# eladb3/SViT

Measured on NVIDIA B200. Metric: clips/sec (16x224^2, bf16) SViT forward, higher is better.
Workload: dtype bf16

## Files before the change

svit_b200/csrc/pool_ln_tiled.cu:

```cuda
#include <cstdlib>
#include <type_traits>

#include "tc_common.cuh"

namespace {

constexpr int PD = 96;
constexpr int TAPS = 27;

struct Geom {
  int B, h, T, H, W, Ho, Wo, O, s;
  int64_t in_bs, in_ts, in_hs;
};

__device__ __forceinline__ float lo_f(uint32_t w) { return __uint_as_float(w << 16); }
__device__ __forceinline__ float hi_f(uint32_t w) { return __uint_as_float(w & 0xffff0000u); }
__device__ __forceinline__ uint32_t pack2(float a, float b) {
  __nv_bfloat162 v = __floats2bfloat162_rn(a, b);
  return *reinterpret_cast<uint32_t*>(&v);
}
__device__ __forceinline__ float half_sum(float v) {
  const unsigned mask = 0xffffu << (threadIdx.x & 16);
#pragma unroll
  for (int o = 8; o > 0; o >>= 1) v += __shfl_xor_sync(mask, v, o);
// ... 392 lines not shown
      if (ho0 + srow >= g.Ho || nvalid < 0) nvalid = 0;
      const int64_t row0 = ((int64_t)bh * Nout + 1 + (int64_t)(ho0 + srow) * g.Wo + wo0 + scol) * PD;
      optr = reinterpret_cast<uint32_t*>(out + row0) + wd;
      if (SAVE) pptr = reinterpret_cast<uint32_t*>(pre + row0) + wd;
    }
    if (g.T == 1) {
      step(R0{}, EONLY{}, 0);
    } else {
      step(R0{}, EFIRST{}, 0);
      int tp = 1;
      for (; tp + 3 <= g.T - 1; tp += 3) {
        step(R1{}, EMID{}, tp);
        step(R2{}, EMID{}, tp + 1);
        step(R0{}, EMID{}, tp + 2);
      }
      const int rem = g.T - 1 - tp;
      if (rem == 0) {
        step(R1{}, ELAST{}, tp);
      } else if (rem == 1) {
        step(R1{}, EMID{}, tp);
        step(R2{}, ELAST{}, tp + 1);
      } else {
        step(R1{}, EMID{}, tp);
        step(R2{}, EMID{}, tp + 1);
        step(R0{}, ELAST{}, tp + 2);
      }
    }
  }

  {
    float2* stg = reinterpret_cast<float2*>(ring);
    long long* stg_tok = reinterpret_cast<long long*>(smem + C::NTOK * MK_PITCH * 8);
    float* sweff = aff + 2 * PD;
    const int nbh = g.B * g.h;
    bool have_weff = false;
    for (int item = gridDim.x - 1 - blockIdx.x; item < nbh; item += gridDim.x) {
      if (!have_weff) {
        if (threadIdx.x < 48) {
          float2 a = make_float2(0.f, 0.f);
#pragma unroll
          for (int tp = 0; tp < TAPS; ++tp) {
            const float f = __ldg(frac + tp);
            a.x = fmaf(sw2[tp * 48 + wd].x, f, a.x);
            a.y = fmaf(sw2[tp * 48 + wd].y, f, a.y);
          }
          sweff[2 * wd] = a.x;
          sweff[2 * wd + 1] = a.y;
        }
        have_weff = true;
      }
      const int head = item % g.h, b = item / g.h;
      const bf16* zin = in + (int64_t)b * g.in_bs + (int64_t)head * g.in_hs;
      bf16* obase = out + (int64_t)item * Nout * PD;
      for (int base = 0; base < 1 + g.O; base += C::NTOK) {
        __syncthreads();
        const int n = min(C::NTOK, 1 + g.O - base);
        for (int i = threadIdx.x; i < n * 48; i += MK_THREADS) {
          const int k = i / 48, ww = i - k * 48;
          const int r = base + k;
          const int64_t tok_in = r == 0 ? 0 : L + r;
          const uint32_t v = reinterpret_cast<const uint32_t*>(zin + tok_in * g.in_ts)[ww];
          const float sx = r == 0 ? 1.f : sweff[2 * ww], sy = r == 0 ? 1.f : sweff[2 * ww + 1];
          stg[k * MK_PITCH + ww] = make_float2(lo_f(v) * sx, hi_f(v) * sy);
          if (ww == 0) stg_tok[k] = r == 0 ? 0 : Lo + r;
        }
        __syncthreads();
        mk_ln_flush(stg, stg_tok, aff, n, eps, obase, threadIdx.x, SAVE ? pre + (int64_t)item * Nout * PD : nullptr);
      }
    }
  }
}

__global__ void __launch_bounds__(256, 4)
pool_ln_direct_kernel(const bf16* __restrict__ in, Geom g, const float* __restrict__ w, const float* __restrict__ frac,
                      const float* __restrict__ gamma, const float* __restrict__ beta, bf16* __restrict__ out, float eps,
                      int mode, bf16* __restrict__ pre) {
  __shared__ float sw[TAPS * PD];
  __shared__ float sweff[PD];
  for (int i = threadIdx.x; i < PD * TAPS; i += blockDim.x) sw[(i % TAPS) * PD + i / TAPS] = w[i];
  __syncthreads();
  for (int c = threadIdx.x; c < PD; c += blockDim.x) {
    float a = 0.f;
    for (int t = 0; t < TAPS; ++t) a += sw[t * PD + c] * frac[t];
    sweff[c] = a;
  }
  __syncthreads();
  const int lane = threadIdx.x & 31, l16 = lane & 15;
  float gm[6], bt[6];
  load_affine(gamma, beta, l16, gm, bt);
  const int64_t Lo = (int64_t)g.T * g.Ho * g.Wo, L = (int64_t)g.T * g.H * g.W;
  const int64_t Nout = 1 + Lo + g.O;
  const int64_t per_bh = mode == 0 ? Nout : (int64_t)1 + g.O;
  const int64_t total = (int64_t)g.B * g.h * per_bh;
  const int64_t hw_per_grid = (int64_t)gridDim.x * (blockDim.x >> 4);
  for (int64_t i = (int64_t)blockIdx.x * (blockDim.x >> 4) + (threadIdx.x >> 4); i < total; i += hw_per_grid) {
    const int64_t r = i % per_bh;
    const int64_t tok = mode == 0 ? r : (r == 0 ? 0 : Lo + r);
    const int head = (int)((i / per_bh) % g.h);
    const int b = (int)(i / (per_bh * g.h));
    const bf16* zin = in + (int64_t)b * g.in_bs + (int64_t)head * g.in_hs;
    float v[6] = {0.f, 0.f, 0.f, 0.f, 0.f, 0.f};
    if (tok == 0 || tok > Lo) {
      const uint32_t* p = reinterpret_cast<const uint32_t*>(zin + (tok == 0 ? 0 : (tok - Lo + L)) * g.in_ts);
#pragma unroll
      for (int j = 0; j < 3; ++j) {
        const uint32_t wd = p[l16 + 16 * j];
        const int c = 2 * (l16 + 16 * j);
        v[2 * j] = lo_f(wd) * (tok == 0 ? 1.f : sweff[c]);
        v[2 * j + 1] = hi_f(wd) * (tok == 0 ? 1.f : sweff[c + 1]);
      }
    } else {
      const int64_t pp = tok - 1;
      const int wo = (int)(pp % g.Wo), ho = (int)((pp / g.Wo) % g.Ho), to = (int)(pp / ((int64_t)g.Wo * g.Ho));
#pragma unroll
      for (int kt = 0; kt < 3; ++kt) {
        const int t = to - 1 + kt;
        if (t < 0 || t >= g.T) continue;
        uint32_t xw[9][3];
#pragma unroll
        for (int kh = 0; kh < 3; ++kh) {
          const int hh = ho * g.s - 1 + kh;
#pragma unroll
          for (int kw = 0; kw < 3; ++kw) {
            const int ww = wo * g.s - 1 + kw;
            const bool ok = hh >= 0 && hh < g.H && ww >= 0 && ww < g.W;
            const uint32_t* q = reinterpret_cast<const uint32_t*>(
                zin + (ok ? (1 + ((int64_t)t * g.H + hh) * g.W + ww) * g.in_ts : 0));
#pragma unroll
            for (int j = 0; j < 3; ++j) xw[kh * 3 + kw][j] = ok ? __ldg(q + l16 + 16 * j) : 0u;
          }
        }
#pragma unroll
        for (int tap = 0; tap < 9; ++tap) {
          const float* wr = sw + (kt * 9 + tap) * PD;
#pragma unroll
          for (int j = 0; j < 3; ++j) {
            const float2 f = *reinterpret_cast<const float2*>(wr + 2 * (l16 + 16 * j));
            v[2 * j] = fmaf(lo_f(xw[tap][j]), f.x, v[2 * j]);
            v[2 * j + 1] = fmaf(hi_f(xw[tap][j]), f.y, v[2 * j + 1]);
          }
        }
      }
    }
    uint32_t* dst = reinterpret_cast<uint32_t*>(out + (((int64_t)b * g.h + head) * Nout + tok) * PD);
    if (pre) {
      uint32_t* pd = reinterpret_cast<uint32_t*>(pre + (((int64_t)b * g.h + head) * Nout + tok) * PD);
#pragma unroll
      for (int j = 0; j < 3; ++j) pd[l16 + 16 * j] = pack2(v[2 * j], v[2 * j + 1]);
    }
    ln_store(v, gm, bt, eps, dst, l16);
  }
}

}

#ifdef SVIT_TIMELINE
extern "C" int svit_debug_pool_timeline(void* device_buffer) {
  unsigned long long* p = (unsigned long long*)device_buffer;
  return (int)cudaMemcpyToSymbol(g_pool_dbg, &p, sizeof(p));
}
#endif

namespace {
template <int SV, int SPRV, bool PERSIST, bool SAVE>
int launch_march(const void* in, int64_t in_bs, int64_t in_ts, const Geom& g, const float* conv_w, const float* tap_frac,
                 const float* gamma, const float* beta, void* out, float eps, cudaStream_t st, void* pre) {
  using C = MkCfg<SV, SPRV>;
  svit_tmap_encode_fn enc = svit_get_tmap_encode();
  if (!enc) return SVIT_ENOTSUP;
  CUtensorMap tm;
  cuuint64_t dims[5] = {(cuuint64_t)g.h * PD, (cuuint64_t)g.W, (cuuint64_t)g.H, (cuuint64_t)g.T, (cuuint64_t)g.B};
  cuuint64_t strides[4] = {(cuuint64_t)in_ts * 2, (cuuint64_t)g.W * in_ts * 2, (cuuint64_t)g.H * g.W * in_ts * 2, (cuuint64_t)in_bs * 2};
  cuuint32_t box[5] = {PD, (cuuint32_t)C::IW, (cuuint32_t)C::IH, 1, 1};
  cuuint32_t estr[5] = {1, 1, 1, 1, 1};
  const bf16* base = (const bf16*)in + in_ts;
  if (enc(&tm, CU_TENSOR_MAP_DATA_TYPE_BFLOAT16, 5, const_cast<bf16*>(base), dims, strides, box, estr,
          CU_TENSOR_MAP_INTERLEAVE_NONE, CU_TENSOR_MAP_SWIZZLE_NONE, CU_TENSOR_MAP_L2_PROMOTION_L2_256B,
          CU_TENSOR_MAP_FLOAT_OOB_FILL_NONE) != CUDA_SUCCESS)
    return SVIT_EINVAL;
  auto kern = pool_ln_march_kernel<SV, SPRV, PERSIST, SAVE>;
  static SvitDevOnce configured;
  if (configured.need()) {
    SVIT_CUDA(cudaFuncSetAttribute(kern, cudaFuncAttributeMaxDynamicSharedMemorySize, C::SMEM));
    configured.done();
  }
  const int tiles = ((g.Wo + C::TW - 1) / C::TW) * ((g.Ho + C::ROWS - 1) / C::ROWS);
  const int64_t ncols = (int64_t)tiles * g.h * g.B;
  if (ncols > (1ll << 30)) return SVIT_EINVAL;
  int64_t grid = PERSIST ? (int64_t)svit_num_sms() * 2 : ncols;
  if (grid > ncols) grid = ncols;
  kern<<<(unsigned)grid, MK_THREADS, C::SMEM, st>>>(tm, (const bf16*)in, g, conv_w, tap_frac, gamma, beta, (bf16*)out, eps,
                                                    tiles, (int)ncols, (bf16*)pre);
  SVIT_CHECK_LAUNCH();
  return 0;
}
}

int svit_pool_ln_fwd_bf16(const void* in, int64_t in_bs, int64_t in_ts, int64_t in_hs, const float* conv_w,
                          const float* tap_frac, const float* gamma, const float* beta, void* out, int B, int h, int T,
                          int H, int W, int O, int s, float eps, cudaStream_t st, void* pre) {
  Geom g;
  g.B = B; g.h = h; g.T = T; g.H = H; g.W = W; g.O = O; g.s = s;
  g.Ho = (H - 1) / s + 1; g.Wo = (W - 1) / s + 1;
  g.in_bs = in_bs; g.in_ts = in_ts; g.in_hs = in_hs;
  const int sms = svit_num_sms();
  const bool tma_ok = (s == 1 || s == 2) && (in_ts % 8 == 0) && (in_bs % 8 == 0) && in_hs == PD && (T * H * W) > 0 &&
                      ((reinterpret_cast<uintptr_t>(in) & 15) == 0) && ((reinterpret_cast<uintptr_t>(out) & 15) == 0);
  if (tma_ok) {
    static const int mode = []() { const char* e = getenv("SVIT_POOL_PERSIST"); return e ? atoi(e) : -1; }();
    const bool wide = s == 1 && g.Wo > 7;
    const int64_t cols_s2 = (int64_t)((g.Wo + 6) / 7) * ((g.Ho + 3) / 4) * h * B;
    const bool persist = mode < 0 ? (s == 2 && cols_s2 >= (int64_t)sms * 12) : mode != 0;
#define MARCH(SV, SPRV)                                                                                               \
  (pre ? (persist ? launch_march<SV, SPRV, true, true>(in, in_bs, in_ts, g, conv_w, tap_frac, gamma, beta, out, eps, st, pre)    \
                  : launch_march<SV, SPRV, false, true>(in, in_bs, in_ts, g, conv_w, tap_frac, gamma, beta, out, eps, st, pre)) \
       : (persist ? launch_march<SV, SPRV, true, false>(in, in_bs, in_ts, g, conv_w, tap_frac, gamma, beta, out, eps, st, nullptr) \
                  : launch_march<SV, SPRV, false, false>(in, in_bs, in_ts, g, conv_w, tap_frac, gamma, beta, out, eps, st, nullptr)))
    if (s == 2) return MARCH(2, 2);
    if (!wide) return MARCH(1, 1);
    return MARCH(1, 2);
#undef MARCH
  }
  const int64_t total = (int64_t)B * h * (1 + (int64_t)T * g.Ho * g.Wo + O);
  int64_t blocks = (total + 15) / 16;
  if (blocks > (int64_t)sms * 16) blocks = (int64_t)sms * 16;
  if (blocks < 1) blocks = 1;
  pool_ln_direct_kernel<<<(unsigned)blocks, 256, 0, st>>>((const bf16*)in, g, conv_w, tap_frac, gamma, beta, (bf16*)out, eps, 0, (bf16*)pre);
  SVIT_CHECK_LAUNCH();
  return 0;
}
```

svit_b200/csrc/stream_bf16.cu:

```cuda
#include "common.cuh"

namespace {

__device__ __forceinline__ void unpack4(uint2 v, float f[4]) {
  f[0] = __uint_as_float(v.x << 16); f[1] = __uint_as_float(v.x & 0xffff0000u);
  f[2] = __uint_as_float(v.y << 16); f[3] = __uint_as_float(v.y & 0xffff0000u);
}
__device__ __forceinline__ uint32_t pack2(float a, float b) {
  __nv_bfloat162 v = __floats2bfloat162_rn(a, b);
  return *reinterpret_cast<uint32_t*>(&v);
}

template <int G, int NQ>
__global__ void __launch_bounds__(256) layernorm_bf16_kernel(const bf16* __restrict__ x, const float* __restrict__ gamma,
                                                             const float* __restrict__ beta, bf16* __restrict__ y,
                                                             float* __restrict__ mean_out, float* __restrict__ rstd_out,
                                                             int64_t rows, float eps) {
  constexpr int C = 4 * G * NQ;
  const int lg = threadIdx.x % G;
  const int64_t group = ((int64_t)blockIdx.x * blockDim.x + threadIdx.x) / G;
  const int64_t ngroups = (int64_t)gridDim.x * blockDim.x / G;
  float gm[NQ][4], bt[NQ][4];
#pragma unroll
  for (int q = 0; q < NQ; ++q) {
    const float4 g4 = *reinterpret_cast<const float4*>(gamma + 4 * (lg + G * q));
    const float4 b4 = *reinterpret_cast<const float4*>(beta + 4 * (lg + G * q));
    gm[q][0] = g4.x; gm[q][1] = g4.y; gm[q][2] = g4.z; gm[q][3] = g4.w;
    bt[q][0] = b4.x; bt[q][1] = b4.y; bt[q][2] = b4.z; bt[q][3] = b4.w;
  }
  const int64_t iters = (rows + ngroups - 1) / ngroups;
  for (int64_t it = 0; it < iters; ++it) {
    const int64_t row = group + it * ngroups;
    const bool ok = row < rows;
    float v[NQ][4];
    float s = 0.f;
#pragma unroll
    for (int q = 0; q < NQ; ++q) {
      uint2 raw = make_uint2(0u, 0u);
      if (ok) raw = *reinterpret_cast<const uint2*>(x + row * C + 4 * (lg + G * q));
      unpack4(raw, v[q]);
      s += v[q][0] + v[q][1] + v[q][2] + v[q][3];
    }
#pragma unroll
    for (int o = G / 2; o > 0; o >>= 1) s += __shfl_xor_sync(0xffffffffu, s, o);
    const float mean = s * (1.f / C);
    float qq = 0.f;
#pragma unroll
    for (int q = 0; q < NQ; ++q)
#pragma unroll
      for (int i = 0; i < 4; ++i) {
        v[q][i] -= mean;
        qq += v[q][i] * v[q][i];
      }
#pragma unroll
    for (int o = G / 2; o > 0; o >>= 1) qq += __shfl_xor_sync(0xffffffffu, qq, o);
    const float rstd = rsqrtf(qq * (1.f / C) + eps);
    if (ok) {
#pragma unroll
      for (int q = 0; q < NQ; ++q) {
        uint2 o2;
        o2.x = pack2(v[q][0] * rstd * gm[q][0] + bt[q][0], v[q][1] * rstd * gm[q][1] + bt[q][1]);
        o2.y = pack2(v[q][2] * rstd * gm[q][2] + bt[q][2], v[q][3] * rstd * gm[q][3] + bt[q][3]);
        *reinterpret_cast<uint2*>(y + row * C + 4 * (lg + G * q)) = o2;
      }
      if (lg == 0 && mean_out) {
        mean_out[row] = mean;
        rstd_out[row] = rstd;
      }
    }
  }
}

template <typename TI>
__global__ void __launch_bounds__(256) im2col_rows_kernel(const TI* __restrict__ x, bf16* __restrict__ cols, int Cin, int T,
                                                          int H, int W, int To, int Ho, int Wo, int kt, int kh, int kw,
                                                          int st, int sh, int sw, int pt, int ph, int pw, int Kpad, int RW) {
  extern __shared__ __align__(16) unsigned char smem_raw[];
  const int R = Cin * kt * kh;
  bf16* rows = reinterpret_cast<bf16*>(smem_raw);
  int* koff = reinterpret_cast<int*>(smem_raw + (((size_t)R * RW * 2 + 15) & ~size_t(15)));
  const int ho = blockIdx.x % Ho, to = (blockIdx.x / Ho) % To, b = blockIdx.x / (Ho * To);
  const int K = R * kw;
  for (int k = threadIdx.x; k < Kpad; k += blockDim.x) koff[k] = k < K ? (k / kw) * RW + (k % kw) : -1;
  for (int i = threadIdx.x; i < R * RW; i += blockDim.x) {
    const int r = i / RW, col = i % RW;
    const int dh = r % kh, dt = (r / kh) % kt, c = r / (kh * kt);
    const int t = to * st - pt + dt, hh = ho * sh - ph + dh, ww = col - pw;
    float v = 0.f;
    if (t >= 0 && t < T && hh >= 0 && hh < H && ww >= 0 && ww < W)
      v = to_f(x[((((int64_t)b * Cin + c) * T + t) * H + hh) * W + ww]);
    rows[i] = __float2bfloat16_rn(v);
  }
  __syncthreads();
  const int cpr = Kpad >> 3;
  bf16* obase = cols + ((((int64_t)b * To + to) * Ho + ho) * Wo) * Kpad;
  const unsigned short* rs = reinterpret_cast<const unsigned short*>(rows);
  for (int i = threadIdx.x; i < Wo * cpr; i += blockDim.x) {
    const int wo = i / cpr, q = i % cpr;
    const int base = wo * sw;
    unsigned short e[8];
#pragma unroll
    for (int u = 0; u < 8; ++u) {
      const int off = koff[q * 8 + u];
      e[u] = off < 0 ? (unsigned short)0 : rs[off + base];
    }
    uint4 o;
    o.x = e[0] | ((uint32_t)e[1] << 16); o.y = e[2] | ((uint32_t)e[3] << 16);
    o.z = e[4] | ((uint32_t)e[5] << 16); o.w = e[6] | ((uint32_t)e[7] << 16);
    *reinterpret_cast<uint4*>(obase + (int64_t)wo * Kpad + q * 8) = o;
  }
}

constexpr int IM_HALO = 4;
__global__ void __launch_bounds__(256) im2col_rows_vec_kernel(const bf16* __restrict__ x, bf16* __restrict__ cols, int Cin,
                                                              int T, int H, int W, int To, int Ho, int Wo, int kt, int kh,
                                                              int kw, int st, int sh, int sw, int pt, int ph, int pw,
                                                              int Kpad, int RW) {
  extern __shared__ __align__(16) unsigned char smem_raw[];
  unsigned short* rows = reinterpret_cast<unsigned short*>(smem_raw);
  const int R = Cin * kt * kh, K = R * kw;
  const int ho = blockIdx.x % Ho, to = (blockIdx.x / Ho) % To, b = blockIdx.x / (Ho * To);
  const int cpr = Kpad >> 3, wchunks = W >> 3;
  for (int i = threadIdx.x; i < R * (wchunks + 2); i += blockDim.x) {
    const int r = i / (wchunks + 2), j = i % (wchunks + 2) - 1;
    unsigned short* dst = rows + r * RW;
    if (j < 0) {
      *reinterpret_cast<uint2*>(dst) = make_uint2(0u, 0u);
    } else if (j == wchunks) {
      *reinterpret_cast<uint2*>(dst + IM_HALO + W) = make_uint2(0u, 0u);
    } else {
      const int dh = r % kh, dt = (r / kh) % kt, c = r / (kh * kt);
      const int t = to * st - pt + dt, hh = ho * sh - ph + dh;
      uint4 v = make_uint4(0u, 0u, 0u, 0u);
      if (t >= 0 && t < T && hh >= 0 && hh < H)
        v = __ldg(reinterpret_cast<const uint4*>(x + ((((int64_t)b * Cin + c) * T + t) * H + hh) * W + 8 * j));
      uint2* d2 = reinterpret_cast<uint2*>(dst + IM_HALO + 8 * j);
      d2[0] = make_uint2(v.x, v.y);
      d2[1] = make_uint2(v.z, v.w);
    }
  }
  const int q = threadIdx.x % cpr, w_first = threadIdx.x / cpr, w_step = blockDim.x / cpr;
  int off[8];
#pragma unroll
  for (int u = 0; u < 8; ++u) {
    const int k = q * 8 + u;
    off[u] = k < K ? (k / kw) * RW + (k % kw) + IM_HALO - pw : -1;
  }
  __syncthreads();
  bf16* obase = cols + ((((int64_t)b * To + to) * Ho + ho) * Wo) * Kpad + q * 8;
  for (int wo = w_first; wo < Wo; wo += w_step) {
    const int base = wo * sw;
    unsigned short e[8];
#pragma unroll
    for (int u = 0; u < 8; ++u) e[u] = off[u] < 0 ? (unsigned short)0 : rows[off[u] + base];
    uint4 o;
    o.x = e[0] | ((uint32_t)e[1] << 16); o.y = e[2] | ((uint32_t)e[3] << 16);
    o.z = e[4] | ((uint32_t)e[5] << 16); o.w = e[6] | ((uint32_t)e[7] << 16);
    *reinterpret_cast<uint4*>(obase + (int64_t)wo * Kpad) = o;
  }
}

template <bool IDX>
__global__ void __launch_bounds__(256) skip_maxpool_bf16_kernel(const bf16* __restrict__ x, bf16* __restrict__ y,
                                                                uint8_t* __restrict__ idx, int B, int C,
                                                                int T_, int H, int W, int Ho, int Wo, int O, int s) {
  const int C8 = C >> 3;
  const int64_t Lin = (int64_t)T_ * H * W, Lout = (int64_t)T_ * Ho * Wo;
  const int64_t Nin = 1 + Lin + O, Nout = 1 + Lout + O;
  const int64_t total = (int64_t)B * Nout * C8;
  for (int64_t i = (int64_t)blockIdx.x * blockDim.x + threadIdx.x; i < total; i += (int64_t)gridDim.x * blockDim.x) {
    const int c8 = (int)(i % C8);
    const int64_t r = i / C8;
    const int64_t tok = r % Nout;
    const int b = (int)(r / Nout);
    const bf16* xb = x + (int64_t)b * Nin * C + c8 * 8;
    uint4 o;
    if (tok == 0) {
      o = *reinterpret_cast<const uint4*>(xb);
    } else if (tok > Lout) {
      o = *reinterpret_cast<const uint4*>(xb + (tok - Lout + Lin) * C);
    } else {
      const int64_t p = tok - 1;
      const int wo = (int)(p % Wo), ho = (int)((p / Wo) % Ho), t = (int)(p / ((int64_t)Wo * Ho));
      uint4 taps[9];
      bool ok[9];
#pragma unroll
      for (int dh = 0; dh < 3; ++dh)
#pragma unroll
        for (int dw = 0; dw < 3; ++dw) {
          const int hh = ho * s - 1 + dh, ww = wo * s - 1 + dw;
          ok[dh * 3 + dw] = hh >= 0 && hh < H && ww >= 0 && ww < W;
          taps[dh * 3 + dw] = ok[dh * 3 + dw]
              ? *reinterpret_cast<const uint4*>(xb + (1 + ((int64_t)t * H + hh) * W + ww) * C) : make_uint4(0, 0, 0, 0);
        }
      float m[8];
      uint32_t win[8];
#pragma unroll
      for (int u = 0; u < 8; ++u) { m[u] = -INFINITY; win[u] = 0u; }
#pragma unroll
      for (int k = 0; k < 9; ++k)
        if (ok[k]) {
          const uint32_t wv[4] = {taps[k].x, taps[k].y, taps[k].z, taps[k].w};
#pragma unroll
          for (int u = 0; u < 4; ++u) {
            const float a = __uint_as_float(wv[u] << 16), c = __uint_as_float(wv[u] & 0xffff0000u);
            if (a > m[2 * u] || a != a) { m[2 * u] = a; if (IDX) win[2 * u] = (uint32_t)k; }
            if (c > m[2 * u + 1] || c != c) { m[2 * u + 1] = c; if (IDX) win[2 * u + 1] = (uint32_t)k; }
          }
        }
      o.x = pack2(m[0], m[1]); o.y = pack2(m[2], m[3]); o.z = pack2(m[4], m[5]); o.w = pack2(m[6], m[7]);
      if (IDX) {
        uint2 iv;
        iv.x = win[0] | (win[1] << 8) | (win[2] << 16) | (win[3] << 24);
        iv.y = win[4] | (win[5] << 8) | (win[6] << 16) | (win[7] << 24);
        *reinterpret_cast<uint2*>(idx + ((int64_t)b * Nout + tok) * C + c8 * 8) = iv;
      }
    }
    *reinterpret_cast<uint4*>(y + ((int64_t)b * Nout + tok) * C + c8 * 8) = o;
  }
}

__global__ void __launch_bounds__(256) skip_maxpool_bwd_idx_kernel(const uint8_t* __restrict__ idx, const bf16* __restrict__ dy,
                                                                   bf16* __restrict__ dx, int B, int C, int T_, int H, int W,
                                                                   int Ho, int Wo, int O, int s) {
  const int C8 = C >> 3;
  const int64_t Lin = (int64_t)T_ * H * W, Lout = (int64_t)T_ * Ho * Wo;
  const int64_t Nin = 1 + Lin + O, Nout = 1 + Lout + O;
  const int64_t total = (int64_t)B * Nin * C8;
  for (int64_t i = (int64_t)blockIdx.x * blockDim.x + threadIdx.x; i < total; i += (int64_t)gridDim.x * blockDim.x) {
    const int c = (int)(i % C8) * 8;
    const int64_t r = i / C8;
    const int64_t tok = r % Nin;
    const int b = (int)(r / Nin);
    const bf16* dyb = dy + (int64_t)b * Nout * C + c;
    const uint8_t* ib = idx + (int64_t)b * Nout * C + c;
    bf16* o = dx + r * C + c;
    if (tok == 0) {
      *reinterpret_cast<uint4*>(o) = __ldg(reinterpret_cast<const uint4*>(dyb));
      continue;
    }
    if (tok > Lin) {
      *reinterpret_cast<uint4*>(o) = __ldg(reinterpret_cast<const uint4*>(dyb + (tok - Lin + Lout) * C));
      continue;
    }
    const int64_t p = tok - 1;
    const int w = (int)(p % W), h = (int)((p / W) % H), t = (int)(p / ((int64_t)W * H));
    float g[8] = {0.f, 0.f, 0.f, 0.f, 0.f, 0.f, 0.f, 0.f};
    for (int ho = (h - 1 + s - 1) / s; ho * s <= h + 1 && ho < Ho; ++ho) {
      if (ho < 0) continue;
      const int dh = h - (ho * s - 1);
      for (int wo = (w - 1 + s - 1) / s; wo * s <= w + 1 && wo < Wo; ++wo) {
        if (wo < 0) continue;
        const uint32_t me = (uint32_t)(dh * 3 + (w - (wo * s - 1)));
        const int64_t orow = 1 + ((int64_t)t * Ho + ho) * Wo + wo;
        const uint2 iv = __ldg(reinterpret_cast<const uint2*>(ib + orow * C));
        const uint32_t hit_lo = iv.x ^ (me * 0x01010101u), hit_hi = iv.y ^ (me * 0x01010101u);
        if (((hit_lo - 0x01010101u) & ~hit_lo & 0x80808080u) | ((hit_hi - 0x01010101u) & ~hit_hi & 0x80808080u)) {
          const uint4 dv = __ldg(reinterpret_cast<const uint4*>(dyb + orow * C));
          const uint32_t wv[4] = {dv.x, dv.y, dv.z, dv.w};
#pragma unroll
          for (int u = 0; u < 4; ++u) {
            const uint32_t b0 = ((u < 2 ? hit_lo : hit_hi) >> (16 * (u & 1))) & 0xffu;
            const uint32_t b1 = ((u < 2 ? hit_lo : hit_hi) >> (16 * (u & 1) + 8)) & 0xffu;
            if (b0 == 0u) g[2 * u] += __uint_as_float(wv[u] << 16);
            if (b1 == 0u) g[2 * u + 1] += __uint_as_float(wv[u] & 0xffff0000u);
          }
        }
      }
    }
    uint4 ov;
    ov.x = pack2(g[0], g[1]); ov.y = pack2(g[2], g[3]); ov.z = pack2(g[4], g[5]); ov.w = pack2(g[6], g[7]);
    *reinterpret_cast<uint4*>(o) = ov;
  }
}

}

extern "C" int svit_skip_maxpool_fwd_idx(const void* x, void* y, void* idx, int B, int C, int T, int H, int W, int O,
                                         int stride_hw, int dtype, void* stream) {
  if (!x || !y || !idx || stride_hw < 2 || B < 0 || O < 1) return SVIT_EINVAL;
  if (dtype != SVIT_BF16 || C % 8 ||
      ((reinterpret_cast<uintptr_t>(x) | reinterpret_cast<uintptr_t>(y)) & 15) || (reinterpret_cast<uintptr_t>(idx) & 7))
    return SVIT_ENOTSUP;
  const int Ho = (H - 1) / stride_hw + 1, Wo = (W - 1) / stride_hw + 1;
  const int64_t total = (int64_t)B * (1 + (int64_t)T * Ho * Wo + O) * (C / 8);
  if (total == 0) return 0;
  int64_t blocks = (total + 255) / 256;
  if (blocks > (int64_t)svit_num_sms() * 32) blocks = (int64_t)svit_num_sms() * 32;
  skip_maxpool_bf16_kernel<true><<<(unsigned)blocks, 256, 0, (cudaStream_t)stream>>>((const bf16*)x, (bf16*)y, (uint8_t*)idx, B, C,
                                                                                   T, H, W, Ho, Wo, O, stride_hw);
  SVIT_CHECK_LAUNCH();
  return 0;
}

extern "C" int svit_skip_maxpool_bwd_idx(const void* idx, const void* dy, void* dx, int B, int C, int T, int H, int W, int O,
                                         int stride_hw, int dtype, void* stream) {
  if (!idx || !dy || !dx || stride_hw < 2 || B < 0 || O < 1) return SVIT_EINVAL;
  if (dtype != SVIT_BF16 || C % 8 ||
      ((reinterpret_cast<uintptr_t>(dy) | reinterpret_cast<uintptr_t>(dx)) & 15) || (reinterpret_cast<uintptr_t>(idx) & 7))
    return SVIT_ENOTSUP;
  const int Ho = (H - 1) / stride_hw + 1, Wo = (W - 1) / stride_hw + 1;
  const int64_t total = (int64_t)B * (1 + (int64_t)T * H * W + O) * (C / 8);
  if (total == 0) return 0;
  int64_t blocks = (total + 255) / 256;
  if (blocks > (int64_t)svit_num_sms() * 32) blocks = (int64_t)svit_num_sms() * 32;
  skip_maxpool_bwd_idx_kernel<<<(unsigned)blocks, 256, 0, (cudaStream_t)stream>>>((const uint8_t*)idx, (const bf16*)dy, (bf16*)dx, B,
                                                                                C, T, H, W, Ho, Wo, O, stride_hw);
  SVIT_CHECK_LAUNCH();
  return 0;
}

int svit_skip_maxpool_fwd_bf16(const void* x, void* y, int B, int C, int T, int H, int W, int Ho, int Wo, int O, int s,
                               cudaStream_t st) {
  if (C % 8 || (reinterpret_cast<uintptr_t>(x) & 15) || (reinterpret_cast<uintptr_t>(y) & 15)) return 0;
  const int64_t total = (int64_t)B * (1 + (int64_t)T * Ho * Wo + O) * (C / 8);
  int64_t blocks = (total + 255) / 256;
  if (blocks > (int64_t)svit_num_sms() * 32) blocks = (int64_t)svit_num_sms() * 32;
  skip_maxpool_bf16_kernel<false><<<(unsigned)blocks, 256, 0, st>>>((const bf16*)x, (bf16*)y, nullptr, B, C, T, H, W, Ho, Wo, O, s);
  cudaError_t e = cudaGetLastError();
  return e == cudaSuccess ? 1 : 1000 + (int)e;
}

int svit_layernorm_fwd_bf16(const void* x, const float* gamma, const float* beta, void* y, float* mean, float* rstd,
                            int64_t rows, int C, float eps, cudaStream_t st) {
  if ((reinterpret_cast<uintptr_t>(x) & 7) || (reinterpret_cast<uintptr_t>(y) & 7) ||
      (reinterpret_cast<uintptr_t>(gamma) & 15) || (reinterpret_cast<uintptr_t>(beta) & 15))
    return 0;
  const int sms = svit_num_sms();
#define LN_LAUNCH(G, NQ)                                                                                           \
  {                                                                                                                \
    int64_t blocks = (rows * G + 255) / 256;                                                                       \
    if (blocks > (int64_t)sms * 16) blocks = (int64_t)sms * 16;                                                    \
    layernorm_bf16_kernel<G, NQ><<<(unsigned)blocks, 256, 0, st>>>((const bf16*)x, gamma, beta, (bf16*)y, mean, rstd, \
                                                                  rows, eps);                                      \
  }
  if (C == 96) LN_LAUNCH(8, 3)
  else if (C == 192) LN_LAUNCH(16, 3)
  else if (C == 384) LN_LAUNCH(32, 3)
  else if (C == 768) LN_LAUNCH(32, 6)
  else return 0;
#undef LN_LAUNCH
  cudaError_t e = cudaGetLastError();
  return e == cudaSuccess ? 1 : 1000 + (int)e;
}

int svit_im2col_rows(const void* x, void* cols, int B, int Cin, int T, int H, int W, int To, int Ho, int Wo, int kt, int kh,
                     int kw, int st_, int sh, int sw, int pt, int ph, int pw, int Kpad, int in_dtype, cudaStream_t st) {
  if (Kpad % 8 || (reinterpret_cast<uintptr_t>(cols) & 15)) return 0;
  const int R = Cin * kt * kh;
  const int RW = (W + 2 * pw + 1) & ~1;
  if ((Wo - 1) * sw + kw > RW) return 0;
  const size_t smem = (((size_t)R * RW * 2 + 15) & ~size_t(15)) + (size_t)Kpad * 4;
  if (smem > 200 * 1024) return 0;
  const unsigned grid = (unsigned)((int64_t)B * To * Ho);
  cudaError_t e;
  const int cpr = Kpad / 8;
  if (in_dtype == SVIT_BF16 && W % 8 == 0 && pw <= IM_HALO && cpr <= 64 && (reinterpret_cast<uintptr_t>(x) & 15) == 0) {
    const int RWv = (W + 2 * IM_HALO + 7) & ~7;
    const int threads = (256 / cpr) * cpr;
    const size_t smv = (size_t)R * RWv * 2;
    if ((Wo - 1) * sw + kw - 1 - pw < W + 4 && smv <= 200 * 1024) {
      static size_t confv = 0;
      if (smv > confv) {
        if ((e = cudaFuncSetAttribute(im2col_rows_vec_kernel, cudaFuncAttributeMaxDynamicSharedMemorySize, (int)smv)) != cudaSuccess)
          return 1000 + (int)e;
        confv = smv;
      }
      im2col_rows_vec_kernel<<<grid, threads, smv, st>>>((const bf16*)x, (bf16*)cols, Cin, T, H, W, To, Ho, Wo, kt, kh, kw, st_,
                                                         sh, sw, pt, ph, pw, Kpad, RWv);
      e = cudaGetLastError();
      return e == cudaSuccess ? 1 : 1000 + (int)e;
    }
  }
  if (in_dtype == SVIT_BF16) {
    static size_t conf = 0;
    if (smem > conf) {
      if ((e = cudaFuncSetAttribute(im2col_rows_kernel<bf16>, cudaFuncAttributeMaxDynamicSharedMemorySize, (int)smem)) != cudaSuccess)
        return 1000 + (int)e;
      conf = smem;
    }
    im2col_rows_kernel<bf16><<<grid, 256, smem, st>>>((const bf16*)x, (bf16*)cols, Cin, T, H, W, To, Ho, Wo, kt, kh, kw, st_,
                                                      sh, sw, pt, ph, pw, Kpad, RW);
  } else {
    static size_t conf = 0;
    if (smem > conf) {
      if ((e = cudaFuncSetAttribute(im2col_rows_kernel<float>, cudaFuncAttributeMaxDynamicSharedMemorySize, (int)smem)) != cudaSuccess)
        return 1000 + (int)e;
      conf = smem;
    }
    im2col_rows_kernel<float><<<grid, 256, smem, st>>>((const float*)x, (bf16*)cols, Cin, T, H, W, To, Ho, Wo, kt, kh, kw,
                                                       st_, sh, sw, pt, ph, pw, Kpad, RW);
  }
  e = cudaGetLastError();
  return e == cudaSuccess ? 1 : 1000 + (int)e;
}


template <typename OT>
__global__ void __launch_bounds__(256) normalize_u8_kernel(const uint8_t* __restrict__ in, OT* __restrict__ out, int64_t npix16,
                                                           int64_t THW, float m0, float m1, float m2, float s0, float s1,
                                                           float s2) {
  const float mean[3] = {m0, m1, m2}, sd[3] = {s0, s1, s2};
  for (int64_t i = (int64_t)blockIdx.x * blockDim.x + threadIdx.x; i < npix16; i += (int64_t)gridDim.x * blockDim.x) {
    const int64_t pix = i * 16;
    const int64_t b = pix / THW, r = pix - b * THW;
    const uint4* src = reinterpret_cast<const uint4*>(in + pix * 3);
    const uint4 q0 = __ldg(src), q1 = __ldg(src + 1), q2 = __ldg(src + 2);
    const uint32_t w[12] = {q0.x, q0.y, q0.z, q0.w, q1.x, q1.y, q1.z, q1.w, q2.x, q2.y, q2.z, q2.w};
    float v[3][16];
#pragma unroll
    for (int k = 0; k < 48; ++k) {
      const float f = (float)((w[k >> 2] >> ((k & 3) * 8)) & 255u);
      const int c = k % 3;
      v[c][k / 3] = __fdiv_rn(__fsub_rn(__fdiv_rn(f, 255.0f), mean[c]), sd[c]);
    }
#pragma unroll
    for (int c = 0; c < 3; ++c) {
      OT* dst = out + (b * 3 + c) * THW + r;
      if (sizeof(OT) == 2) {
        uint32_t o[8];
#pragma unroll
        for (int k = 0; k < 8; ++k) {
          __nv_bfloat162 h = __floats2bfloat162_rn(v[c][2 * k], v[c][2 * k + 1]);
          o[k] = *reinterpret_cast<uint32_t*>(&h);
        }
        reinterpret_cast<uint4*>(dst)[0] = make_uint4(o[0], o[1], o[2], o[3]);
        reinterpret_cast<uint4*>(dst)[1] = make_uint4(o[4], o[5], o[6], o[7]);
      } else {
#pragma unroll
        for (int k = 0; k < 4; ++k)
          reinterpret_cast<float4*>(dst)[k] = make_float4(v[c][4 * k], v[c][4 * k + 1], v[c][4 * k + 2], v[c][4 * k + 3]);
      }
    }
  }
}

extern "C" int svit_normalize_u8(const void* frames, void* out, int B, int T, int H, int W, float mean0, float mean1,
                                 float mean2, float std0, float std1, float std2, int out_dtype, void* stream) {
  if (!frames || !out || B < 0 || T < 1 || H < 1 || W < 1) return SVIT_EINVAL;
  const int64_t THW = (int64_t)T * H * W;
  if (THW % 16 || (reinterpret_cast<uintptr_t>(frames) & 15) || (reinterpret_cast<uintptr_t>(out) & 15)) return SVIT_ENOTSUP;
  if (B == 0) return 0;
  const int64_t n16 = (int64_t)B * THW / 16;
  cudaStream_t st = (cudaStream_t)stream;
  int64_t grid = (n16 + 255) / 256;
  const int64_t cap = (int64_t)svit_num_sms() * 16;
  if (grid > cap) grid = cap;
  if (out_dtype == SVIT_BF16)
    normalize_u8_kernel<bf16><<<(unsigned)grid, 256, 0, st>>>((const uint8_t*)frames, (bf16*)out, n16, THW, mean0, mean1, mean2, std0, std1, std2);
  else if (out_dtype == SVIT_F32)
    normalize_u8_kernel<float><<<(unsigned)grid, 256, 0, st>>>((const uint8_t*)frames, (float*)out, n16, THW, mean0, mean1, mean2, std0, std1, std2);
  else
    return SVIT_EINVAL;
  SVIT_CHECK_LAUNCH();
  return 0;
}

template <typename OT>
__global__ void __launch_bounds__(256) crop_flip_normalize_u8_kernel(const uint8_t* __restrict__ in, OT* __restrict__ out,
                                                                     const int32_t* __restrict__ x_off,
                                                                     const int32_t* __restrict__ y_off,
                                                                     const int32_t* __restrict__ flip, int64_t nquads, int T,
                                                                     int H, int W, int cs_h, int cs_w, float m0, float m1,
                                                                     float m2, float s0, float s1, float s2) {
  const float mean[3] = {m0, m1, m2}, sd[3] = {s0, s1, s2};
  const int qw = cs_w >> 2;
  for (int64_t i = (int64_t)blockIdx.x * blockDim.x + threadIdx.x; i < nquads; i += (int64_t)gridDim.x * blockDim.x) {
    const int q = (int)(i % qw);
    int64_t r = i / qw;
    const int y = (int)(r % cs_h);
    r /= cs_h;
// ... 210 lines not shown
```

Baseline: 3199.

## Add strided pool+LN kernel with temporal reuse and banded skip maxpool

Adds a dedicated pool+LayerNorm kernel for spatial strides of three or more. It walks time per output column and keeps three rolling accumulators, so each input frame is loaded once and feeds all three temporal taps. Weights are held in shared memory, and the cls and extra tokens are handled by folding the effective tap weights. The skip maxpool kernel is also restructured so each thread computes a vertical band of four output rows and reuses overlapping tap rows when the stride is two, with special tokens split into a separate index range. The aim is fewer redundant global loads and less index arithmetic, at the cost of fewer, heavier threads and a non-persistent grid.

```diff
diff --git a/svit_b200/csrc/pool_ln_tiled.cu b/svit_b200/csrc/pool_ln_tiled.cu
--- a/svit_b200/csrc/pool_ln_tiled.cu
+++ b/svit_b200/csrc/pool_ln_tiled.cu
@@ -568,6 +568,100 @@
   }
 }
 
+__device__ __forceinline__ void strided_emit(const float v[6], const float gm[6], const float bt[6], float eps, bf16* out,
+                                             bf16* pre, int64_t row, int l16) {
+  if (pre) {
+    uint32_t* pd = reinterpret_cast<uint32_t*>(pre + row * PD);
+#pragma unroll
+    for (int j = 0; j < 3; ++j) pd[l16 + 16 * j] = pack2(v[2 * j], v[2 * j + 1]);
+  }
+  ln_store(v, gm, bt, eps, reinterpret_cast<uint32_t*>(out + row * PD), l16);
+}
+
+__global__ void __launch_bounds__(128)
+pool_ln_strided_kernel(const bf16* __restrict__ in, Geom g, const float* __restrict__ w, const float* __restrict__ frac,
+                       const float* __restrict__ gamma, const float* __restrict__ beta, bf16* __restrict__ out, float eps,
+                       bf16* __restrict__ pre, int ncols, int total) {
+  __shared__ __align__(8) float sw[TAPS * PD];
+  __shared__ float sweff[PD];
+  for (int i = threadIdx.x; i < PD * TAPS; i += blockDim.x) sw[(i % TAPS) * PD + i / TAPS] = w[i];
+  __syncthreads();
+  for (int c = threadIdx.x; c < PD; c += blockDim.x) {
+    float a = 0.f;
+    for (int t = 0; t < TAPS; ++t) a += sw[t * PD + c] * frac[t];
+    sweff[c] = a;
+  }
+  __syncthreads();
+  const int l16 = threadIdx.x & 15;
+  float gm[6], bt[6];
+  load_affine(gamma, beta, l16, gm, bt);
+  const int HoWo = g.Ho * g.Wo, Lo = g.T * HoWo, L = g.T * g.H * g.W, HW = g.H * g.W;
+  const int Nout = 1 + Lo + g.O;
+  const int step = gridDim.x * (blockDim.x >> 4);
+  for (int i = blockIdx.x * (blockDim.x >> 4) + (threadIdx.x >> 4); i < total; i += step) {
+    if (i >= ncols) {
+      const int j = i - ncols, r = j % (1 + g.O), bh = j / (1 + g.O);
+      const int head = bh % g.h, b = bh / g.h;
+      const int tok = r == 0 ? 0 : Lo + r;
+      const uint32_t* p = reinterpret_cast<const uint32_t*>(in + (int64_t)b * g.in_bs + (int64_t)head * g.in_hs +
+                                                            (int64_t)(r == 0 ? 0 : L + r) * g.in_ts);
+      float v[6];
+#pragma unroll
+      for (int j3 = 0; j3 < 3; ++j3) {
+        const uint32_t wd = p[l16 + 16 * j3];
+        const int c = 2 * (l16 + 16 * j3);
+        v[2 * j3] = lo_f(wd) * (r == 0 ? 1.f : sweff[c]);
+        v[2 * j3 + 1] = hi_f(wd) * (r == 0 ? 1.f : sweff[c + 1]);
+      }
+      strided_emit(v, gm, bt, eps, out, pre, (int64_t)bh * Nout + tok, l16);
+      continue;
+    }
+    const int col = i % HoWo, bh = i / HoWo;
+    const int ho = col / g.Wo, wo = col - ho * g.Wo;
+    const int head = bh % g.h, b = bh / g.h;
+    const uint32_t* zin = reinterpret_cast<const uint32_t*>(in + (int64_t)b * g.in_bs + (int64_t)head * g.in_hs) + l16;
+    const int64_t orow = (int64_t)bh * Nout + 1 + col;
+    int toff[9];
+#pragma unroll
+    for (int kh = 0; kh < 3; ++kh)
+#pragma unroll
+      for (int kw = 0; kw < 3; ++kw) {
+        const int hh = ho * g.s - 1 + kh, ww = wo * g.s - 1 + kw;
+        toff[kh * 3 + kw] = hh >= 0 && hh < g.H && ww >= 0 && ww < g.W ? hh * g.W + ww : -1;
+      }
+    float a0[6], a1[6], a2[6];
+#pragma unroll
+    for (int u = 0; u < 6; ++u) { a0[u] = 0.f; a1[u] = 0.f; a2[u] = 0.f; }
+    for (int t = 0; t < g.T; ++t) {
+      const uint32_t* zt = zin + (int64_t)(1 + t * HW) * (g.in_ts >> 1);
+      uint32_t xw[9][3];
+#pragma unroll
+      for (int k = 0; k < 9; ++k)
+#pragma unroll
+        for (int j = 0; j < 3; ++j)
+          xw[k][j] = toff[k] >= 0 ? __ldg(zt + (int64_t)toff[k] * (g.in_ts >> 1) + 16 * j) : 0u;
+#pragma unroll
+      for (int tap = 0; tap < 9; ++tap) {
+#pragma unroll
+        for (int j = 0; j < 3; ++j) {
+          const int c = 2 * (l16 + 16 * j);
+          const float x0 = lo_f(xw[tap][j]), x1 = hi_f(xw[tap][j]);
+          const float2 f2 = *reinterpret_cast<const float2*>(sw + (18 + tap) * PD + c);
+          const float2 f1 = *reinterpret_cast<const float2*>(sw + (9 + tap) * PD + c);
+          const float2 f0 = *reinterpret_cast<const float2*>(sw + tap * PD + c);
+          a0[2 * j] = fmaf(x0, f2.x, a0[2 * j]); a0[2 * j + 1] = fmaf(x1, f2.y, a0[2 * j + 1]);
+          a1[2 * j] = fmaf(x0, f1.x, a1[2 * j]); a1[2 * j + 1] = fmaf(x1, f1.y, a1[2 * j + 1]);
+          a2[2 * j] = fmaf(x0, f0.x, a2[2 * j]); a2[2 * j + 1] = fmaf(x1, f0.y, a2[2 * j + 1]);
+        }
+      }
+      if (t > 0) strided_emit(a0, gm, bt, eps, out, pre, orow + (int64_t)(t - 1) * HoWo, l16);
+#pragma unroll
+      for (int u = 0; u < 6; ++u) { a0[u] = a1[u]; a1[u] = a2[u]; a2[u] = 0.f; }
+    }
+    strided_emit(a0, gm, bt, eps, out, pre, orow + (int64_t)(g.T - 1) * HoWo, l16);
+  }
+}
+
 }
 
 #ifdef SVIT_TIMELINE
@@ -641,6 +735,15 @@
   int64_t blocks = (total + 15) / 16;
   if (blocks > (int64_t)sms * 16) blocks = (int64_t)sms * 16;
   if (blocks < 1) blocks = 1;
+  const int64_t ncols = (int64_t)B * h * g.Ho * g.Wo, nitems = ncols + (int64_t)B * h * (1 + O);
+  const bool strided_ok = s >= 3 && T >= 1 && in_ts % 8 == 0 && ((reinterpret_cast<uintptr_t>(in) & 15) == 0) &&
+                          nitems < (1ll << 31) && (int64_t)T * H * W < (1ll << 31);
+  if (strided_ok) {
+    pool_ln_strided_kernel<<<(unsigned)((nitems + 7) / 8), 128, 0, st>>>((const bf16*)in, g, conv_w, tap_frac, gamma, beta,
+                                                                         (bf16*)out, eps, (bf16*)pre, (int)ncols, (int)nitems);
+    SVIT_CHECK_LAUNCH();
+    return 0;
+  }
   pool_ln_direct_kernel<<<(unsigned)blocks, 256, 0, st>>>((const bf16*)in, g, conv_w, tap_frac, gamma, beta, (bf16*)out, eps, 0, (bf16*)pre);
   SVIT_CHECK_LAUNCH();
   return 0;
diff --git a/svit_b200/csrc/stream_bf16.cu b/svit_b200/csrc/stream_bf16.cu
--- a/svit_b200/csrc/stream_bf16.cu
+++ b/svit_b200/csrc/stream_bf16.cu
@@ -160,64 +160,94 @@
   }
 }
 
+constexpr int SKIP_BAND = 4;
+
 template <bool IDX>
 __global__ void __launch_bounds__(256) skip_maxpool_bf16_kernel(const bf16* __restrict__ x, bf16* __restrict__ y,
-                                                                uint8_t* __restrict__ idx, int B, int C,
-                                                                int T_, int H, int W, int Ho, int Wo, int O, int s) {
+                                                                uint8_t* __restrict__ idx, int C, int T_, int H, int W,
+                                                                int Ho, int Wo, int O, int s, int nband, int n_pool,
+                                                                int n_total) {
+  const int i = blockIdx.x * blockDim.x + threadIdx.x;
+  if (i >= n_total) return;
   const int C8 = C >> 3;
   const int64_t Lin = (int64_t)T_ * H * W, Lout = (int64_t)T_ * Ho * Wo;
   const int64_t Nin = 1 + Lin + O, Nout = 1 + Lout + O;
-  const int64_t total = (int64_t)B * Nout * C8;
-  for (int64_t i = (int64_t)blockIdx.x * blockDim.x + threadIdx.x; i < total; i += (int64_t)gridDim.x * blockDim.x) {
-    const int c8 = (int)(i % C8);
-    const int64_t r = i / C8;
-    const int64_t tok = r % Nout;
-    const int b = (int)(r / Nout);
-    const bf16* xb = x + (int64_t)b * Nin * C + c8 * 8;
+  if (i >= n_pool) {
+    const int j = i - n_pool, c8 = j % C8, r = j / C8, k = r % (1 + O), b = r / (1 + O);
+    const int64_t tin = k == 0 ? 0 : Lin + k, tout = k == 0 ? 0 : Lout + k;
+    *reinterpret_cast<uint4*>(y + ((int64_t)b * Nout + tout) * C + c8 * 8) =
+        *reinterpret_cast<const uint4*>(x + ((int64_t)b * Nin + tin) * C + c8 * 8);
+    return;
+  }
+  const int c8 = i % C8;
+  int r = i / C8;
+  const int wo = r % Wo;
+  r /= Wo;
+  const int band = r % nband;
+  r /= nband;
+  const int t = r % T_, b = r / T_;
+  const bf16* xp = x + ((int64_t)b * Nin + 1 + (int64_t)t * H * W) * C + c8 * 8;
+  const int64_t orow0 = (int64_t)b * Nout + 1 + (int64_t)t * Ho * Wo + wo;
+  bool okc[3];
+#pragma unroll
+  for (int dw = 0; dw < 3; ++dw) okc[dw] = wo * s - 1 + dw >= 0 && wo * s - 1 + dw < W;
+  const int ho0 = band * SKIP_BAND, ho1 = min(ho0 + SKIP_BAND, Ho);
+  uint4 taps[9];
+  bool ok[9];
+  for (int ho = ho0; ho < ho1; ++ho) {
+    const bool carry = s == 2 && ho > ho0;
+#pragma unroll
+    for (int dh = 0; dh < 3; ++dh) {
+      if (dh == 0 && carry) {
+#pragma unroll
+        for (int dw = 0; dw < 3; ++dw) { taps[dw] = taps[6 + dw]; ok[dw] = ok[6 + dw]; }
+        continue;
+      }
+      const int hh = ho * s - 1 + dh;
+      const bool okr = hh >= 0 && hh < H;
+#pragma unroll
+      for (int dw = 0; dw < 3; ++dw) {
+        const int k = dh * 3 + dw;
+        ok[k] = okr && okc[dw];
+        taps[k] = ok[k] ? __ldg(reinterpret_cast<const uint4*>(xp + ((int64_t)hh * W + wo * s - 1 + dw) * C))
+                        : make_uint4(0, 0, 0, 0);
+      }
+    }
+    float m[8];
+    uint32_t win[8];
+#pragma unroll
+    for (int u = 0; u < 8; ++u) { m[u] = -INFINITY; win[u] = 0u; }
+#pragma unroll
+    for (int k = 0; k < 9; ++k)
+      if (ok[k]) {
+        const uint32_t wv[4] = {taps[k].x, taps[k].y, taps[k].z, taps[k].w};
+#pragma unroll
+        for (int u = 0; u < 4; ++u) {
+          const float a = __uint_as_float(wv[u] << 16), c = __uint_as_float(wv[u] & 0xffff0000u);
+          if (a > m[2 * u] || a != a) { m[2 * u] = a; if (IDX) win[2 * u] = (uint32_t)k; }
+          if (c > m[2 * u + 1] || c != c) { m[2 * u + 1] = c; if (IDX) win[2 * u + 1] = (uint32_t)k; }
+        }
+      }
     uint4 o;
-    if (tok == 0) {
-      o = *reinterpret_cast<const uint4*>(xb);
-    } else if (tok > Lout) {
-      o = *reinterpret_cast<const uint4*>(xb + (tok - Lout + Lin) * C);
-    } else {
-      const int64_t p = tok - 1;
-      const int wo = (int)(p % Wo), ho = (int)((p / Wo) % Ho), t = (int)(p / ((int64_t)Wo * Ho));
-      uint4 taps[9];
-      bool ok[9];
-#pragma unroll
-      for (int dh = 0; dh < 3; ++dh)
-#pragma unroll
-        for (int dw = 0; dw < 3; ++dw) {
-          const int hh = ho * s - 1 + dh, ww = wo * s - 1 + dw;
-          ok[dh * 3 + dw] = hh >= 0 && hh < H && ww >= 0 && ww < W;
-          taps[dh * 3 + dw] = ok[dh * 3 + dw]
-              ? *reinterpret_cast<const uint4*>(xb + (1 + ((int64_t)t * H + hh) * W + ww) * C) : make_uint4(0, 0, 0, 0);
-        }
-      float m[8];
-      uint32_t win[8];
-#pragma unroll
-      for (int u = 0; u < 8; ++u) { m[u] = -INFINITY; win[u] = 0u; }
-#pragma unroll
-      for (int k = 0; k < 9; ++k)
-        if (ok[k]) {
-          const uint32_t wv[4] = {taps[k].x, taps[k].y, taps[k].z, taps[k].w};
-#pragma unroll
-          for (int u = 0; u < 4; ++u) {
-            const float a = __uint_as_float(wv[u] << 16), c = __uint_as_float(wv[u] & 0xffff0000u);
-            if (a > m[2 * u] || a != a) { m[2 * u] = a; if (IDX) win[2 * u] = (uint32_t)k; }
-            if (c > m[2 * u + 1] || c != c) { m[2 * u + 1] = c; if (IDX) win[2 * u + 1] = (uint32_t)k; }
-          }
-        }
-      o.x = pack2(m[0], m[1]); o.y = pack2(m[2], m[3]); o.z = pack2(m[4], m[5]); o.w = pack2(m[6], m[7]);
-      if (IDX) {
-        uint2 iv;
-        iv.x = win[0] | (win[1] << 8) | (win[2] << 16) | (win[3] << 24);
-        iv.y = win[4] | (win[5] << 8) | (win[6] << 16) | (win[7] << 24);
-        *reinterpret_cast<uint2*>(idx + ((int64_t)b * Nout + tok) * C + c8 * 8) = iv;
-      }
-    }
-    *reinterpret_cast<uint4*>(y + ((int64_t)b * Nout + tok) * C + c8 * 8) = o;
-  }
+    o.x = pack2(m[0], m[1]); o.y = pack2(m[2], m[3]); o.z = pack2(m[4], m[5]); o.w = pack2(m[6], m[7]);
+    const int64_t orow = orow0 + (int64_t)ho * Wo;
+    if (IDX) {
+      uint2 iv;
+      iv.x = win[0] | (win[1] << 8) | (win[2] << 16) | (win[3] << 24);
+      iv.y = win[4] | (win[5] << 8) | (win[6] << 16) | (win[7] << 24);
+      *reinterpret_cast<uint2*>(idx + orow * C + c8 * 8) = iv;
+    }
+    *reinterpret_cast<uint4*>(y + orow * C + c8 * 8) = o;
+  }
+}
+
+bool skip_items(int B, int C, int T, int Ho, int Wo, int O, int& nband, int& n_pool, int& n_total) {
+  nband = (Ho + SKIP_BAND - 1) / SKIP_BAND;
+  const int64_t p = (int64_t)B * T * nband * Wo * (C / 8), t = p + (int64_t)B * (1 + O) * (C / 8);
+  if (t >= (1ll << 31) - 256) return false;
+  n_pool = (int)p;
+  n_total = (int)t;
+  return true;
 }
 
 __global__ void __launch_bounds__(256) skip_maxpool_bwd_idx_kernel(const uint8_t* __restrict__ idx, const bf16* __restrict__ dy,
@@ -283,12 +313,11 @@
       ((reinterpret_cast<uintptr_t>(x) | reinterpret_cast<uintptr_t>(y)) & 15) || (reinterpret_cast<uintptr_t>(idx) & 7))
     return SVIT_ENOTSUP;
   const int Ho = (H - 1) / stride_hw + 1, Wo = (W - 1) / stride_hw + 1;
-  const int64_t total = (int64_t)B * (1 + (int64_t)T * Ho * Wo + O) * (C / 8);
-  if (total == 0) return 0;
-  int64_t blocks = (total + 255) / 256;
-  if (blocks > (int64_t)svit_num_sms() * 32) blocks = (int64_t)svit_num_sms() * 32;
-  skip_maxpool_bf16_kernel<true><<<(unsigned)blocks, 256, 0, (cudaStream_t)stream>>>((const bf16*)x, (bf16*)y, (uint8_t*)idx, B, C,
-                                                                                   T, H, W, Ho, Wo, O, stride_hw);
+  int nband, n_pool, n_total;
+  if (!skip_items(B, C, T, Ho, Wo, O, nband, n_pool, n_total)) return SVIT_ENOTSUP;
+  if (n_total == 0) return 0;
+  skip_maxpool_bf16_kernel<true><<<(unsigned)((n_total + 255) / 256), 256, 0, (cudaStream_t)stream>>>(
+      (const bf16*)x, (bf16*)y, (uint8_t*)idx, C, T, H, W, Ho, Wo, O, stride_hw, nband, n_pool, n_total);
   SVIT_CHECK_LAUNCH();
   return 0;
 }
@@ -313,10 +342,11 @@
 int svit_skip_maxpool_fwd_bf16(const void* x, void* y, int B, int C, int T, int H, int W, int Ho, int Wo, int O, int s,
                                cudaStream_t st) {
   if (C % 8 || (reinterpret_cast<uintptr_t>(x) & 15) || (reinterpret_cast<uintptr_t>(y) & 15)) return 0;
-  const int64_t total = (int64_t)B * (1 + (int64_t)T * Ho * Wo + O) * (C / 8);
-  int64_t blocks = (total + 255) / 256;
-  if (blocks > (int64_t)svit_num_sms() * 32) blocks = (int64_t)svit_num_sms() * 32;
-  skip_maxpool_bf16_kernel<false><<<(unsigned)blocks, 256, 0, st>>>((const bf16*)x, (bf16*)y, nullptr, B, C, T, H, W, Ho, Wo, O, s);
+  int nband, n_pool, n_total;
+  if (!skip_items(B, C, T, Ho, Wo, O, nband, n_pool, n_total)) return 0;
+  if (n_total == 0) return 1;
+  skip_maxpool_bf16_kernel<false><<<(unsigned)((n_total + 255) / 256), 256, 0, st>>>(
+      (const bf16*)x, (bf16*)y, nullptr, C, T, H, W, Ho, Wo, O, s, nband, n_pool, n_total);
   cudaError_t e = cudaGetLastError();
   return e == cudaSuccess ? 1 : 1000 + (int)e;
 }
```

Result: faster. 3267 (median of 6 runs) (+2.1%).
